# Shashank8834/multimodal-fl-security

Hardware: AMD Instinct MI355X
Metric: FL rounds/sec + aggregate-ms, K=128 clients 10M-param multimodal, 1/2/4/8 GPU (higher is better)
Workload: dtype f32 (bf16x6-split MFMA conv/GEMM = fp32 operands; Krum Gram bf16x4 hi/lo split, fp32 accumulate); 1 GPU; C3: Multi-Krum K=128, 20% sign-flip, ResNet-18 img + 1-layer GRU text late fusion, 5 local SGD steps/round; Krum distances reference-exact; preset=C3, model=resnet18-img+gru1-text late-fusion, clients=128, params=11800394, local_steps=5, batch=32, defense=krum(f=25, multi_k=64), attack=sign_flip, attackers=25, client_chunk=128, exchange=alltoall, krum_distances=reference-exact (fp32 torch.norm accumulation, D bit-identical to krum.py:89-97), training_phase=one captured HIP graph per round; local updates = one flr_train_clients_ex call

## Files before the change

### include/flr.h

```cpp
#ifndef FLR_H
#define FLR_H

#include <stddef.h>
#include <stdint.h>

#ifdef __cplusplus
extern "C" {
#endif

#define FLR_OK 0
#define FLR_ERR_ARG (-1)
#define FLR_ERR_HIP (-2)
#define FLR_ERR_UNSUPPORTED (-3)
#define FLR_ERR_WORKSPACE (-4)
#define FLR_ERR_KRUM_N (-5)

const char* flr_version(void);
const char* flr_build_info(void);
int flr_set_knob(const char* name, const char* value);
const char* flr_status_string(int status);
const char* flr_last_error(void);

size_t flr_pairwise_l2_workspace(int64_t K, int64_t P);
int flr_pairwise_l2(const float* X, int64_t K, int64_t P, int64_t ldx,
// ... 302 lines not shown
                 double* out, void* workspace, size_t workspace_bytes, void* stream);
int flr_weighted_rows(const float* X, int64_t K, int64_t P, int64_t ldx,
                      const int32_t* rows, int64_t m, const float* weights,
                      const float* scales, float divisor, float* out,
                      void* stream);

int flr_gru_fwd_step(const float* gi, const float* gh, float* hseq, float* gates,
                     int64_t K, int64_t B, int64_t T, int64_t H, int64_t t,
                     void* stream);
int flr_gru_bwd_step(const float* dh, const float* gates, const float* hseq,
                     float* dgh, float* dgi, float* dh_direct, int64_t K,
                     int64_t B, int64_t T, int64_t H, int64_t t, void* stream);
int flr_gru_fwd_fused(const float* gi, const float* whhP, const float* bhh, float* hseq, float* gates, int64_t K,
                      int64_t B, int64_t T, int64_t H, int64_t t, void* stream);
int flr_gru_bwd_fused(const float* whhTP, const float* gates, const float* hseq, float* dgh, float* dgi,
                      float* dh_direct, float* dh0, int64_t K, int64_t B, int64_t T, int64_t H, int64_t t,
                      void* stream);
int flr_gru_fwd_fused_ex(const float* gi, const float* whh, int shared_w, const float* bhh,
                         float* hseq, float* gates, int64_t K, int64_t B, int64_t T, int64_t H,
                         int64_t t, void* stream);
int flr_gru_bwd_fused_ex(const float* whhT, int shared_w, const float* gates, const float* hseq,
                         float* dgh, float* dgi, float* dh_direct, float* dh0, int64_t K,
                         int64_t B, int64_t T, int64_t H, int64_t t, void* stream);
int flr_gru_pack(const float* w, int64_t K, int64_t NG, int64_t H, int64_t C, int trans, float* wp, void* stream);

int flr_batchnorm_fwd(const float* x, const float* gamma, const float* beta,
                      const float* residual, float* y, float* mean, float* invstd,
                      int64_t B, int64_t KC, int64_t HW, float eps, int relu,
                      void* stream);
int flr_batchnorm_bwd(const float* dy, const float* x, const float* y,
                      const float* gamma, const float* mean, const float* invstd,
                      float* dx, float* dgamma, float* dbeta, float* dresidual,
                      int64_t B, int64_t KC, int64_t HW, int relu, void* stream);
int flr_batchnorm_relu_maxpool_fwd(const float* x, const float* gamma, const float* beta,
                                   float* y_pool, uint8_t* argmax, float* mean, float* invstd,
                                   int64_t KC, int64_t NI, int64_t H, int64_t W, float eps,
                                   void* stream);
int flr_maxpool_relu_batchnorm_bwd(const float* dy_pool, const uint8_t* argmax, const float* x,
                                   const float* gamma, const float* beta, const float* mean,
                                   const float* invstd, float* dx, float* dgamma, float* dbeta,
                                   int64_t KC, int64_t NI, int64_t H, int64_t W, void* stream);

size_t flr_bgemm_workspace(int64_t batch, int64_t M, int64_t N, int64_t R);
#define FLR_ACT_NONE 0
#define FLR_ACT_RELU 1
#define FLR_ACT_GELU 2
// ... 113 lines not shown
```

### multimodal-fl-security_amd/csrc/train_clients.hip

```cpp
#include "flr_common.h"
#include "side_stream.h"

#include <algorithm>
#include <cstring>
#include <string>
#include <vector>

namespace flr {
int clip_sumsq_blocks(const float* const* g_blocks, const int64_t* numel, const int64_t* client_stride,
                      int64_t nblocks, int64_t K, double* out, int64_t out_ld, int nslots, hipStream_t st);
namespace tc {

constexpr int THREADS = 256;

__global__ void permute_images_kernel(const float* __restrict__ src, float* __restrict__ dst, int64_t K, int64_t B,
                                      int64_t C, int64_t HW) {
  const int64_t n = K * B * C * HW;
  for (int64_t i = (int64_t)blockIdx.x * THREADS + threadIdx.x; i < n; i += (int64_t)gridDim.x * THREADS) {
    const int64_t p = i % HW, r = i / HW;
    const int64_t b = r % B, r2 = r / B;
    const int64_t c = r2 % C, k = r2 / C;
    dst[i] = src[((k * B + b) * C + c) * HW + p];
  }
}
// ... 451 lines not shown
  int step(const float* images, const int64_t* tokens, const int64_t* labels, const float* mask, bool first,
           bool last, float* loss_row, float lr, float mom, hipStream_t st) {
    int rc;
#define FLR_TRY(x) \
  if ((rc = (x)) != FLR_OK) return rc
    const auto& s = s_;
    const int64_t C0 = s.in_channels, HW0 = s.image_size * s.image_size, N = B_ * T_;
    first_ = first;
    hipLaunchKernelGGL(permute_images_kernel, dim3(grid_for(K_ * B_ * C0 * HW0)), dim3(THREADS), 0, st, images,
                       ximg_, K_, B_, C0, HW0);
    FLR_TRY(launch_status("train_clients: images"));
    const Param &emb = ps_[p_emb_], &wih = ps_[p_wih_], &whh = ps_[p_whh_], &bih = ps_[p_bih_],
                &bhh = ps_[p_bhh_], &w1 = ps_[p_w1_], &b1 = ps_[p_b1_], &w2 = ps_[p_w2_], &b2 = ps_[p_b2_];
    const bool conc = text_ != nullptr;
    const hipStream_t ts = conc ? text_->s : st;
    if (conc) FLR_TRY(fork(st, ts, 0));
    FLR_TRY(wait_group(gtext_, ts));
    FLR_TRY(flr_embedding_fwd(emb.w, s.vocab * E_, s.vocab, tokens, N, nullptr, 0, 0, nullptr, 0, nullptr, 0, 0,
                              nullptr, 0, K_, N, E_, emb_, ts));
    const int64_t H3 = 3 * H_;
    FLR_TRY(gemm(emb_, N * E_, E_, 1, wih.w, H3 * E_, E_, 1, gi_, N * H3, H3, 1, bih.w, H3, nullptr, N, H3, E_, ts));
    const bool fused = B_ <= 32;
    const bool wsh = first_ && gshared_ != nullptr;
    if (fused) {
      FLR_TRY(flr_fill(hseq_, K_ * (T_ + 1) * B_ * H_, 0.f, ts));
      FLR_TRY(flr_gru_pack(wsh ? gshared_ + whh.off : whh.w, wsh ? 1 : K_, 3, H_, H_, 0, whhP_, ts));
      for (int64_t t = 0; t < T_; ++t)
        FLR_TRY(flr_gru_fwd_fused_ex(gi_, whhP_, wsh ? 1 : 0, bhh.w, hseq_, gates_, K_, B_, T_, H_, t, ts));
    } else {
      FLR_TRY(flr_fill(hseq_, K_ * (T_ + 1) * B_ * H_, 0.f, ts));
      for (int64_t t = 0; t < T_; ++t) {
        FLR_TRY(gemm(hseq_ + t * B_ * H_, (T_ + 1) * B_ * H_, H_, 1, whh.w, H3 * H_, H_, 1, gh_, B_ * H3, H3, 1,
                     bhh.w, H3, nullptr, B_, H3, H_, ts));
        FLR_TRY(flr_gru_fwd_step(gi_, gh_, hseq_, gates_, K_, B_, T_, H_, t, ts));
      }
    }
    if (conc) FLR_TRY(fork(ts, st, 1));
    int seg = 0;
    FLR_TRY(wait_group(seg++, st));
    FLR_TRY(conv_fwd(stem_, ximg_, y0_, st));
    if (stem_fused_) {
      FLR_TRY(flr_batchnorm_relu_maxpool_fwd(y0_, ps_[stem_bn_.pg].w, ps_[stem_bn_.pb].w, p0_, arg0_, stem_bn_.mean,
                                             stem_bn_.invstd, K_ * s.widths[0], B_, Hs_, Hs_, 1e-5f, st));
    } else {
      FLR_TRY(bn_fwd(stem_bn_, y0_, nullptr, a0_, true, st));
      FLR_TRY(flr_maxpool2d_fwd(a0_, p0_, arg0_, K_ * s.widths[0] * B_, Hs_, Hs_, 3, 3, 2, 1, st));
    }
// ... 35 lines not shown
    FLR_TRY(flr_bgemm_ex(hT, hk, H_, 1, w1.w + Dimg_, F_ * DI, DI, 1, h1_, B_ * F_, F_, 1, nullptr, 0, h1_,
                         FLR_ACT_RELU, mask, nullptr, nullptr, K_, B_, F_, H_, gws_, gws_n_, st));
    FLR_TRY(gemm(h1_, B_ * F_, F_, 1, w2.w, C_ * F_, F_, 1, logits_, B_ * C_, C_, 1, b2.w, C_, nullptr, B_, C_, F_,
                 st));
    FLR_TRY(flr_cross_entropy(logits_, labels, K_, B_, C_, loss_, dlogits_, rows_, st));
    FLR_TRY(flr_copy_rows(loss_, K_, K_, loss_row, K_, 1, st));
    WgradStream* wgs_save = wgs_;
    wev_ = 0;
    FLR_TRY(flr_bgemm_ex(dlogits_, B_ * C_, C_, 1, w2.w, C_ * F_, 1, F_, dpre_, B_ * F_, F_, 1, nullptr, 0, nullptr,
                         FLR_ACT_DRELU, mask, h1_, nullptr, K_, B_, F_, C_, gws_, gws_n_, st));
    FLR_TRY(gemm(dlogits_, B_ * C_, 1, C_, h1_, B_ * F_, 1, F_, w2.g, C_ * F_, F_, 1, nullptr, 0, nullptr, C_, F_, B_,
                 st));
    FLR_TRY(rowsum(dlogits_, B_ * C_, C_, B_, C_, b2.g, st));
    FLR_TRY(gemm(dpre_, B_ * F_, F_, 1, w1.w, F_ * DI, 1, DI, d_x4_, Dimg_ * B_, 1, B_, nullptr, 0, nullptr, B_, Dimg_,
                 F_, st));
    FLR_TRY(gemm(dpre_, B_ * F_, 1, F_, x4, Dimg_ * B_, B_, 1, w1.g, F_ * DI, DI, 1, nullptr, 0, nullptr, F_, Dimg_, B_,
                 st));
    FLR_TRY(gemm(dpre_, B_ * F_, F_, 1, w1.w + Dimg_, F_ * DI, 1, DI, dh_, B_ * H_, H_, 1, nullptr, 0, nullptr, B_, H_,
                 F_, st));
    FLR_TRY(gemm(dpre_, B_ * F_, 1, F_, hT, hk, 1, H_, w1.g + Dimg_, F_ * DI, DI, 1, nullptr, 0, nullptr, F_, H_, B_,
                 st));
    FLR_TRY(rowsum(dpre_, B_ * F_, F_, B_, F_, b1.g, st));
    if (conc) FLR_TRY(fork(st, ts, 2));
    if (fused) {
      FLR_TRY(flr_gru_pack(wsh ? gshared_ + whh.off : whh.w, wsh ? 1 : K_, 1, H_, H3, 1, whhT_, ts));
      FLR_TRY(flr_gru_bwd_step(dh_, gates_, hseq_, dgh_, dgi_, dh_direct_, K_, B_, T_, H_, T_ - 1, ts));
      for (int64_t t = T_ - 1; t > 0; --t)
        FLR_TRY(flr_gru_bwd_fused_ex(whhT_, wsh ? 1 : 0, gates_, hseq_, dgh_, dgi_, dh_direct_, nullptr, K_, B_, T_,
                                     H_, t, ts));
    } else {
      const float* dh = dh_;
      for (int64_t t = T_ - 1; t >= 0; --t) {
        FLR_TRY(flr_gru_bwd_step(dh, gates_, hseq_, dgh_, dgi_, dh_direct_, K_, B_, T_, H_, t, ts));
        if (t > 0) {
          float* out = dh == dh2_ ? dh_ : dh2_;
          FLR_TRY(gemm(dgh_ + t * B_ * H3, T_ * B_ * H3, H3, 1, whh.w, H3 * H_, 1, H_, out, B_ * H_, H_, 1, nullptr,
                       0, dh_direct_, B_, H_, H3, ts));
          dh = out;
        }
      }
    }
    FLR_TRY(gemm(dgh_, T_ * B_ * H3, 1, H3, hseq_, hk, 1, H_, whh.g, H3 * H_, H_, 1, nullptr, 0, nullptr, H3, H_,
                 T_ * B_, ts));
    FLR_TRY(rowsum(dgh_, T_ * B_ * H3, H3, T_ * B_, H3, bhh.g, ts));
    FLR_TRY(gemm(dgi_, N * H3, H3, 1, wih.w, H3 * E_, 1, E_, demb_, N * E_, E_, 1, nullptr, 0, nullptr, N, E_, H3, ts));
    FLR_TRY(gemm(dgi_, N * H3, 1, H3, emb_, N * E_, 1, E_, wih.g, H3 * E_, E_, 1, nullptr, 0, nullptr, H3, E_, N, ts));
    FLR_TRY(rowsum(dgi_, N * H3, H3, N, H3, bih.g, ts));
// ... 475 lines not shown
```

### multimodal-fl-security_amd/csrc/train_gru.hip

```cpp
#include "flr_common.h"

#include <stdlib.h>
#include <string.h>

namespace flr {
namespace gru {

constexpr int THREADS = 256;

__device__ __forceinline__ float sigm(float x) { return 1.0f / (1.0f + expf(-x)); }

struct Dims {
  int K, B, T, H, t;
  int wshared;
};

__device__ __forceinline__ void decompose(const Dims& d, int64_t idx, int& k, int& b, int& j) {
  j = (int)(idx % d.H);
  const int64_t kb = idx / d.H;
  b = (int)(kb % d.B);
  k = (int)(kb / d.B);
}

__global__ __launch_bounds__(THREADS) void fwd_step_kernel(const float* __restrict__ gi, const float* __restrict__ gh,
                                                           float* __restrict__ hseq, float* __restrict__ gates,
                                                           const Dims d) {
  const int64_t idx = (int64_t)blockIdx.x * THREADS + threadIdx.x;
  if (idx >= (int64_t)d.K * d.B * d.H) return;
  int k, b, j;
  decompose(d, idx, k, b, j);
  const int H = d.H;
  const int64_t kb = (int64_t)k * d.B + b;
  const float* gir = gi + (kb * d.T + d.t) * 3 * H;
  const float* ghr = gh + kb * 3 * H;
  const int64_t hrow = (((int64_t)k * (d.T + 1) + d.t) * d.B + b) * H;
  const float hp = hseq[hrow + j];
  const float r = sigm(gir[j] + ghr[j]);
  const float z = sigm(gir[H + j] + ghr[H + j]);
  const float hn = ghr[2 * H + j];
  const float n = tanhf(gir[2 * H + j] + r * hn);
  hseq[hrow + (int64_t)d.B * H + j] = (hp - n) * z + n;
  float* g = gates + (((int64_t)k * d.T + d.t) * d.B + b) * 4 * H;
  g[j] = r;
  g[H + j] = z;
  g[2 * H + j] = n;
  g[3 * H + j] = hn;
}

__global__ __launch_bounds__(THREADS) void bwd_step_kernel(const float* __restrict__ dh,
                                                           const float* __restrict__ gates,
                                                           const float* __restrict__ hseq, float* __restrict__ dgh,
                                                           float* __restrict__ dgi, float* __restrict__ dh_direct,
                                                           const Dims d) {
  const int64_t idx = (int64_t)blockIdx.x * THREADS + threadIdx.x;
  if (idx >= (int64_t)d.K * d.B * d.H) return;
  int k, b, j;
  decompose(d, idx, k, b, j);
  const int H = d.H;
  const int64_t kb = (int64_t)k * d.B + b;
  const int64_t srow = ((int64_t)k * d.T + d.t) * d.B + b;
  const float* g = gates + srow * 4 * H;
  const float r = g[j], z = g[H + j], n = g[2 * H + j], hn = g[3 * H + j];
  const float hp = hseq[(((int64_t)k * (d.T + 1) + d.t) * d.B + b) * H + j];
  const float dy = dh[idx];
  const float dz = dy * (hp - n);
  const float dn = dy * (1.0f - z);
  const float dnp = dn * (1.0f - n * n);
  const float dr = dnp * hn;
  const float drp = dr * (r * (1.0f - r));
  const float dzp = dz * (z * (1.0f - z));
  float* o = dgh + srow * 3 * H;
  o[j] = drp;
  o[H + j] = dzp;
  o[2 * H + j] = dnp * r;
  float* q = dgi + (kb * d.T + d.t) * 3 * H;
  q[j] = drp;
  q[H + j] = dzp;
  q[2 * H + j] = dnp;
  dh_direct[idx] = dy * z;
}

typedef __bf16 bf16x8 __attribute__((ext_vector_type(8)));
typedef float f32x16 __attribute__((ext_vector_type(16)));

__device__ __forceinline__ void split3(const float (&v)[8], bf16x8& hi, bf16x8& mid, bf16x8& lo) {
#pragma unroll
  for (int j = 0; j < 8; ++j) {
    const __bf16 a = (__bf16)v[j];
    const float r1 = v[j] - (float)a;
    const __bf16 b = (__bf16)r1;
    hi[j] = a;
    mid[j] = b;
    lo[j] = (__bf16)(r1 - (float)b);
  }
}

using rsrc_t = __amdgpu_buffer_rsrc_t;
typedef float f32x4 __attribute__((ext_vector_type(4)));
constexpr unsigned SENT = 0x80000000u;

__device__ __forceinline__ rsrc_t make_rsrc(const float* p, int64_t nfloats) {
  const uint64_t a = reinterpret_cast<uint64_t>(p);
  const uint32_t lo = __builtin_amdgcn_readfirstlane((uint32_t)a);
  const uint32_t hi = __builtin_amdgcn_readfirstlane((uint32_t)(a >> 32));
  const int bytes = __builtin_amdgcn_readfirstlane((int)(nfloats * 4));
  void* base = reinterpret_cast<void*>(((uint64_t)hi << 32) | lo);
  return __builtin_amdgcn_make_buffer_rsrc(base, (short)0, bytes, 0x00020000);
}

template <bool V8>
__device__ __forceinline__ void bload8(rsrc_t r, bool ok, int row_off, int k0, int R, float (&v)[8]) {
  if constexpr (V8) {
    const unsigned off = (ok && k0 < R) ? (unsigned)(row_off + k0) * 4u : SENT;
    const f32x4 x = __builtin_bit_cast(f32x4, __builtin_amdgcn_raw_buffer_load_b128(r, off, 0, 0));
    const f32x4 y = __builtin_bit_cast(f32x4, __builtin_amdgcn_raw_buffer_load_b128(r, off + 16u, 0, 0));
    v[0] = x[0]; v[1] = x[1]; v[2] = x[2]; v[3] = x[3];
// ... 114 lines not shown
  } else {
#pragma unroll
    for (int g = 0; g < 3; ++g)
#pragma unroll
      for (int e = 0; e < 16; ++e) red[wave][g][e][lane] = acc[g][e];
    __syncthreads();
  }
#pragma unroll
  for (int i = 0; i < EPT; ++i) {
    const int p = threadIdx.x + 64 * NW * i, e = p >> 6, ln = p & 63;
    const int b = (e & 3) + 8 * (e >> 2) + 4 * (ln >> 5), j = j0 + (ln & 31);
    if (b >= B || j >= H) continue;
    float v[3];
#pragma unroll
    for (int g = 0; g < 3; ++g) {
      float x = red[0][g][e][ln];
      if constexpr (!SEQ)
#pragma unroll
        for (int w = 1; w < NW; ++w) x += red[w][g][e][ln];
      v[g] = x;
    }
    const int64_t hrw = (((int64_t)k * (d.T + 1) + d.t) * B + b) * H;
    const float ghr = pbh[i][0] + v[0], ghz = pbh[i][1] + v[1], hn = pbh[i][2] + v[2];
    const float r = sigm(pgi[i][0] + ghr);
    const float z = sigm(pgi[i][1] + ghz);
    const float n = tanhf(pgi[i][2] + r * hn);
    hseq[hrw + (int64_t)B * H + j] = (php[i] - n) * z + n;
    float* gg = gates + (((int64_t)k * d.T + d.t) * B + b) * 4 * H;
    gg[j] = r;
    gg[H + j] = z;
    gg[2 * H + j] = n;
    gg[3 * H + j] = hn;
  }
}

template <bool V8, int NW, int G, bool SEQ = false>
__global__ __launch_bounds__(64 * NW) __attribute__((amdgpu_waves_per_eu(SEQ ? 6 : 1))) void bwd_fused_kernel(const float* __restrict__ whhTP,
                                                            const float* __restrict__ gates,
                                                            const float* __restrict__ hseq, float* __restrict__ dgh,
                                                            float* __restrict__ dgi, float* __restrict__ dh_direct,
                                                            float* __restrict__ dh0, const Dims d, int nub) {
  constexpr int EPT = 16 / NW;
  __shared__ float red[SEQ ? 1 : NW][16][64];
  int k, ub;
  block_coords(nub, k, ub);
  const int i0 = ub * 32;
  const int wave = threadIdx.x >> 6, lane = threadIdx.x & 63, l32 = lane & 31, h = lane >> 5;
  const int B = d.B, H = d.H, R = 3 * H;
  const int t = d.t + 1;
  const rsrc_t ra = make_rsrc(dgh + ((int64_t)k * d.T + t) * B * R, (int64_t)B * R);
  const int S = (R + 15) / 16, per = (S + NW - 1) / NW;
  const rsrc_t rb = make_rsrc(whhTP + (d.wshared ? 0 : (int64_t)k * nub * S * 512), (int64_t)nub * S * 512);
  const rsrc_t rdd = make_rsrc(dh_direct + (int64_t)k * B * H, (int64_t)B * H);
  const bool elem = d.t >= 0;
// ... 44 lines not shown
#pragma unroll
        for (int e = 0; e < 16; ++e) red[0][e][lane] = w == 0 ? acc[e] : red[0][e][lane] + acc[e];
      __syncthreads();
    }
  } else {
#pragma unroll
    for (int e = 0; e < 16; ++e) red[wave][e][lane] = acc[e];
    __syncthreads();
  }
#pragma unroll
  for (int i = 0; i < EPT; ++i) {
    const int p = threadIdx.x + 64 * NW * i, e = p >> 6, ln = p & 63;
    const int b = (e & 3) + 8 * (e >> 2) + 4 * (ln >> 5), j = i0 + (ln & 31);
    if (b >= B || j >= H) continue;
    float x = red[0][e][ln];
    if constexpr (!SEQ)
#pragma unroll
      for (int w = 1; w < NW; ++w) x += red[w][e][ln];
    const int64_t kb = (int64_t)k * B + b;
    const int64_t idx = kb * H + j;
    const float dy = pdd[i] + x;
    if (dh0) dh0[idx] = dy;
    if (!elem) continue;
    const float r = pg[i][0], z = pg[i][1], n = pg[i][2], hn = pg[i][3];
    const float dz = dy * (php[i] - n);
    const float dn = dy * (1.0f - z);
    const float dnp = dn * (1.0f - n * n);
    const float dr = dnp * hn;
    const float drp = dr * (r * (1.0f - r));
    const float dzp = dz * (z * (1.0f - z));
    const int64_t srow = ((int64_t)k * d.T + d.t) * B + b;
    float* o = dgh + srow * 3 * H;
    o[j] = drp;
    o[H + j] = dzp;
    o[2 * H + j] = dnp * r;
    float* q = dgi + (kb * d.T + d.t) * 3 * H;
    q[j] = drp;
    q[H + j] = dzp;
    q[2 * H + j] = dnp;
    dh_direct[idx] = dy * z;
  }
}

template <int TRANS>
__global__ __launch_bounds__(256) void pack_kernel(const float* __restrict__ w, int NG, int H, int C,
                                                   float* __restrict__ wp) {
  __shared__ float tile[32][129];
  const int k = blockIdx.z, blk = blockIdx.y, c0 = blockIdx.x * 128;
  const int nub = (H + 31) / 32, S = (C + 15) / 16;
  const int g = blk / nub, r0 = (blk % nub) * 32;
  const float* src = w + (int64_t)k * NG * H * C;
  for (int e = threadIdx.x; e < 32 * 128; e += 256) {
    int r, c;
    if (TRANS) { c = e >> 5; r = e & 31; } else { r = e >> 7; c = e & 127; }
    const bool ok = r0 + r < H && c0 + c < C;
    const int64_t off = TRANS ? (int64_t)(c0 + c) * H + r0 + r : ((int64_t)g * H + r0 + r) * C + c0 + c;
    tile[r][c] = ok ? src[off] : 0.f;
  }
  __syncthreads();
  float* dst = wp + ((int64_t)k * NG * nub + blk) * S * 512;
  for (int o = threadIdx.x; o < 8 * 512; o += 256) {
    const int sl = o >> 9, q = (o >> 8) & 1, lane = (o >> 2) & 63, e = o & 3;
    const int s = c0 / 16 + sl;
    if (s < S) dst[(int64_t)s * 512 + q * 256 + lane * 4 + e] = tile[lane & 31][sl * 16 + 8 * (lane >> 5) + 4 * q + e];
  }
}

inline bool dims_ok(int64_t K, int64_t B, int64_t T, int64_t H, int64_t t) {
  return K > 0 && B > 0 && T > 0 && H > 0 && t >= 0 && t < T && K * B * H < (int64_t)1 << 31;
}

}
}

using namespace flr;

extern "C" int flr_gru_fwd_step(const float* gi, const float* gh, float* hseq, float* gates, int64_t K, int64_t B,
                                int64_t T, int64_t H, int64_t t, void* stream) {
  if (!gi || !gh || !hseq || !gates || !gru::dims_ok(K, B, T, H, t)) return FLR_ERR_ARG;
  const gru::Dims d{(int)K, (int)B, (int)T, (int)H, (int)t};
  const int64_t n = K * B * H;
  hipLaunchKernelGGL(gru::fwd_step_kernel, dim3((unsigned)((n + gru::THREADS - 1) / gru::THREADS)),
                     dim3(gru::THREADS), 0, as_stream(stream), gi, gh, hseq, gates, d);
  return launch_status("gru fwd step");
}

extern "C" int flr_gru_bwd_step(const float* dh, const float* gates, const float* hseq, float* dgh, float* dgi,
                                float* dh_direct, int64_t K, int64_t B, int64_t T, int64_t H, int64_t t,
// ... 64 lines not shown
                                 float* dh_direct, float* dh0, int64_t K, int64_t B, int64_t T, int64_t H, int64_t t,
                                 void* stream) {
  return flr_gru_bwd_fused_ex(whhT, 0, gates, hseq, dgh, dgi, dh_direct, dh0, K, B, T, H, t, stream);
}

extern "C" int flr_gru_bwd_fused_ex(const float* whhT, int shared_w, const float* gates, const float* hseq,
                                    float* dgh, float* dgi, float* dh_direct, float* dh0, int64_t K, int64_t B,
                                    int64_t T, int64_t H, int64_t t, void* stream) {
  if (!whhT || !gates || !hseq || !dgh || !dgi || !dh_direct || !gru::dims_ok(K, B, T, H, t) || t < 1 || B > 32 ||
      K > 65535)
    return FLR_ERR_ARG;
  const gru::Dims d{(int)K, (int)B, (int)T, (int)H, (int)(t - 1), shared_w ? 1 : 0};
  const int nub = (int)((H + 31) / 32);
  const int cfg = gru::cfg_index("FLR_GRU_BW", 1);
  if (H % 8 == 0)
    gru::launch_bwd<true>(cfg, dim3((unsigned)(K * nub)), as_stream(stream), whhT, gates, hseq, dgh, dgi, dh_direct,
                          dh0, d, nub);
  else
    gru::launch_bwd<false>(cfg, dim3((unsigned)(K * nub)), as_stream(stream), whhT, gates, hseq, dgh, dgi, dh_direct,
                           dh0, d, nub);
  return launch_status("gru bwd fused");
}

extern "C" int flr_gru_pack(const float* w, int64_t K, int64_t NG, int64_t H, int64_t C, int trans, float* wp,
                            void* stream) {
  if (!w || !wp || K < 1 || K > 65535 || NG < 1 || H < 1 || C < 1 || (trans && NG != 1) ||
      K * NG * H * C >= (int64_t)1 << 31)
    return FLR_ERR_ARG;
  const dim3 grid((unsigned)((C + 127) / 128), (unsigned)(NG * ((H + 31) / 32)), (unsigned)K);
  if (trans)
    hipLaunchKernelGGL(gru::pack_kernel<1>, grid, dim3(256), 0, as_stream(stream), w, (int)NG, (int)H, (int)C, wp);
  else
    hipLaunchKernelGGL(gru::pack_kernel<0>, grid, dim3(256), 0, as_stream(stream), w, (int)NG, (int)H, (int)C, wp);
  return launch_status("gru pack");
}
```

### multimodal-fl-security_amd/flr/_capi.py

```python
from __future__ import annotations

import ctypes
import os
import threading

import torch

_PKG_ROOT = os.path.dirname(os.path.dirname(os.path.abspath(__file__)))
LIB_PATH = os.environ.get("FLR_LIB", os.path.join(_PKG_ROOT, "lib", "libflr.so"))
HEADER_PATH = os.path.join(os.path.dirname(_PKG_ROOT), "include", "flr.h")

FLR_OK = 0
FLR_ERR_ARG = -1
FLR_ERR_HIP = -2
FLR_ERR_UNSUPPORTED = -3
FLR_ERR_WORKSPACE = -4
FLR_ERR_KRUM_N = -5

_c_void_p = ctypes.c_void_p
_i64 = ctypes.c_int64
_size_t = ctypes.c_size_t
_int = ctypes.c_int

SIGNATURES = {
# ... 174 lines not shown
    "flr_layernorm_fwd": (_int, [_c_void_p, _i64, _c_void_p, _i64, _c_void_p, _c_void_p, _c_void_p, _i64, _c_void_p,
                                 _i64, _c_void_p, _c_void_p, _i64, _i64, _i64, ctypes.c_float, _c_void_p]),
    "flr_layernorm_bwd_workspace": (_size_t, [_i64, _i64, _i64]),
    "flr_layernorm_bwd": (_int, [_c_void_p, _i64, _c_void_p, _i64, _c_void_p, _c_void_p, _c_void_p, _c_void_p, _i64,
                                 _c_void_p, _i64, _c_void_p, _c_void_p, _i64, _i64, _i64, _c_void_p, _size_t,
                                 _c_void_p]),
    "flr_vit_tokens": (_int, [_c_void_p, _c_void_p, _c_void_p, _i64, _i64, _i64, _i64, _c_void_p, _c_void_p]),
    "flr_attention_fwd": (_int, [_c_void_p, _i64, _i64, _i64, _i64, _c_void_p, _c_void_p, _c_void_p]),
    "flr_attention_bwd": (_int, [_c_void_p, _c_void_p, _c_void_p, _c_void_p, _i64, _i64, _i64, _i64, _c_void_p,
                                 _c_void_p]),
    "flr_sum_rows": (_int, [_c_void_p, _i64, _i64, _i64, _i64, _i64, _c_void_p, _i64, _c_void_p]),
    "flr_sum_rows_workspace": (_size_t, [_i64, _i64, _i64]),
    "flr_sum_rows_ex": (_int, [_c_void_p, _i64, _i64, _i64, _i64, _i64, _c_void_p, _i64, _c_void_p, _size_t,
                               _c_void_p]),
    "flr_maxpool2d_fwd": (_int, [_c_void_p] * 3 + [_i64] * 7 + [_c_void_p]),
    "flr_maxpool2d_bwd": (_int, [_c_void_p] * 3 + [_i64] * 7 + [_c_void_p]),
    "flr_gru_fwd_step": (_int, [_c_void_p] * 4 + [_i64] * 5 + [_c_void_p]),
    "flr_gru_bwd_step": (_int, [_c_void_p] * 6 + [_i64] * 5 + [_c_void_p]),
    "flr_gru_fwd_fused": (_int, [_c_void_p] * 5 + [_i64] * 5 + [_c_void_p]),
    "flr_gru_bwd_fused": (_int, [_c_void_p] * 7 + [_i64] * 5 + [_c_void_p]),
    "flr_gru_pack": (_int, [_c_void_p, _i64, _i64, _i64, _i64, _int, _c_void_p, _c_void_p]),
    "flr_gru_fwd_fused_ex": (_int, [_c_void_p, _c_void_p, _int] + [_c_void_p] * 3 + [_i64] * 5 + [_c_void_p]),
    "flr_gru_bwd_fused_ex": (_int, [_c_void_p, _int] + [_c_void_p] * 6 + [_i64] * 5 + [_c_void_p]),
    "flr_batchnorm_infer": (_int, [_c_void_p] * 7 + [_i64, _i64, ctypes.c_float, _int, _c_void_p]),
    "flr_classify_rows": (_int, [_c_void_p, _c_void_p, _i64, _i64, _i64, _i64, _c_void_p, _c_void_p, _c_void_p,
                                 _c_void_p]),
}

_lock = threading.Lock()
_lib = None


class FlrError(RuntimeError):

    def __init__(self, fn: str, status: int, detail: str = ""):
        self.status = status
        msg = f"{fn} failed: {status_string(status)} ({status})"
        if detail:
            msg += f": {detail}"
        super().__init__(msg)


def lib() -> ctypes.CDLL:
    global _lib
    if _lib is not None:
        return _lib
    with _lock:
# ... 52 lines not shown
```

Measured before the change: 16.95 rounds/s.

## Fuse GRU time loop into one persistent kernel per client for fwd and bwd

Adds sequence-level GRU forward and backward kernels that run all timesteps inside one block per client. The recurrent state is kept in double-buffered LDS as a bf16 hi/mid/lo split, and the recurrent weights are streamed with software-pipelined buffer loads. This replaces T per-step kernel launches and their global round-trips of the hidden state, and zeroes only h0 rather than filling the whole hseq buffer. It is enabled when K*(H/32) exceeds 768 or when a knob forces it. The trade-off is that each client is limited to one workgroup, which can cap parallelism on small K.

After: 17.32 rounds/s, median of 6. 2.1% higher.

```diff
diff --git a/include/flr.h b/include/flr.h
--- a/include/flr.h
+++ b/include/flr.h
@@ -348,6 +348,14 @@
 int flr_gru_bwd_fused_ex(const float* whhT, int shared_w, const float* gates, const float* hseq,
                          float* dgh, float* dgi, float* dh_direct, float* dh0, int64_t K,
                          int64_t B, int64_t T, int64_t H, int64_t t, void* stream);
+int flr_gru_fwd_seq(const float* gi, const float* whhP, int shared_w, const float* bhh, float* hseq, float* gates,
+                    int64_t K, int64_t B, int64_t T, int64_t H, void* stream);
+int flr_gru_bwd_seq(const float* whhTP, int shared_w, const float* gates, const float* hseq, const float* dh,
+                    float* dgh, float* dgi, float* dh_direct, float* dh0, int64_t K, int64_t B, int64_t T,
+                    int64_t H, void* stream);
+int flr_gru_seq_supported(int64_t K, int64_t B, int64_t T, int64_t H);
+int flr_gru_seq_preferred(int64_t K, int64_t B, int64_t T, int64_t H);
+int flr_gru_zero_h0(float* hseq, int64_t K, int64_t B, int64_t T, int64_t H, void* stream);
 int flr_gru_pack(const float* w, int64_t K, int64_t NG, int64_t H, int64_t C, int trans, float* wp, void* stream);
 
 int flr_batchnorm_fwd(const float* x, const float* gamma, const float* beta,
diff --git a/multimodal-fl-security_amd/csrc/train_clients.hip b/multimodal-fl-security_amd/csrc/train_clients.hip
--- a/multimodal-fl-security_amd/csrc/train_clients.hip
+++ b/multimodal-fl-security_amd/csrc/train_clients.hip
@@ -497,7 +497,12 @@
     FLR_TRY(gemm(emb_, N * E_, E_, 1, wih.w, H3 * E_, E_, 1, gi_, N * H3, H3, 1, bih.w, H3, nullptr, N, H3, E_, ts));
     const bool fused = B_ <= 32;
     const bool wsh = first_ && gshared_ != nullptr;
-    if (fused) {
+    const bool seq = fused && flr_gru_seq_preferred(K_, B_, T_, H_) != 0;
+    if (seq) {
+      FLR_TRY(flr_gru_zero_h0(hseq_, K_, B_, T_, H_, ts));
+      FLR_TRY(flr_gru_pack(wsh ? gshared_ + whh.off : whh.w, wsh ? 1 : K_, 3, H_, H_, 0, whhP_, ts));
+      FLR_TRY(flr_gru_fwd_seq(gi_, whhP_, wsh ? 1 : 0, bhh.w, hseq_, gates_, K_, B_, T_, H_, ts));
+    } else if (fused) {
       FLR_TRY(flr_fill(hseq_, K_ * (T_ + 1) * B_ * H_, 0.f, ts));
       FLR_TRY(flr_gru_pack(wsh ? gshared_ + whh.off : whh.w, wsh ? 1 : K_, 3, H_, H_, 0, whhP_, ts));
       for (int64_t t = 0; t < T_; ++t)
@@ -579,7 +584,11 @@
                  st));
     FLR_TRY(rowsum(dpre_, B_ * F_, F_, B_, F_, b1.g, st));
     if (conc) FLR_TRY(fork(st, ts, 2));
-    if (fused) {
+    if (seq) {
+      FLR_TRY(flr_gru_pack(wsh ? gshared_ + whh.off : whh.w, wsh ? 1 : K_, 1, H_, H3, 1, whhT_, ts));
+      FLR_TRY(flr_gru_bwd_seq(whhT_, wsh ? 1 : 0, gates_, hseq_, dh_, dgh_, dgi_, dh_direct_, nullptr, K_, B_, T_, H_,
+                              ts));
+    } else if (fused) {
       FLR_TRY(flr_gru_pack(wsh ? gshared_ + whh.off : whh.w, wsh ? 1 : K_, 1, H_, H3, 1, whhT_, ts));
       FLR_TRY(flr_gru_bwd_step(dh_, gates_, hseq_, dgh_, dgi_, dh_direct_, K_, B_, T_, H_, T_ - 1, ts));
       for (int64_t t = T_ - 1; t > 0; --t)
diff --git a/multimodal-fl-security_amd/csrc/train_gru.hip b/multimodal-fl-security_amd/csrc/train_gru.hip
--- a/multimodal-fl-security_amd/csrc/train_gru.hip
+++ b/multimodal-fl-security_amd/csrc/train_gru.hip
@@ -9,6 +9,35 @@
 constexpr int THREADS = 256;
 
 __device__ __forceinline__ float sigm(float x) { return 1.0f / (1.0f + expf(-x)); }
+
+struct Gate {
+  float r, z, n, h;
+};
+__device__ __forceinline__ Gate gate_math(float gir, float giz, float gin, float ghr, float ghz, float hn, float hp) {
+  Gate o;
+  o.r = sigm(gir + ghr);
+  o.z = sigm(giz + ghz);
+  o.n = tanhf(gin + o.r * hn);
+  o.h = (hp - o.n) * o.z + o.n;
+  return o;
+}
+
+struct ElemBwd {
+  float drp, dzp, dnp, dnr, dhd;
+};
+__device__ __forceinline__ ElemBwd elem_bwd(float dy, float r, float z, float n, float hn, float hp) {
+  const float dz = dy * (hp - n);
+  const float dn = dy * (1.0f - z);
+  const float dnp = dn * (1.0f - n * n);
+  const float dr = dnp * hn;
+  ElemBwd o;
+  o.drp = dr * (r * (1.0f - r));
+  o.dzp = dz * (z * (1.0f - z));
+  o.dnp = dnp;
+  o.dnr = dnp * r;
+  o.dhd = dy * z;
+  return o;
+}
 
 struct Dims {
   int K, B, T, H, t;
@@ -35,15 +64,13 @@
   const float* ghr = gh + kb * 3 * H;
   const int64_t hrow = (((int64_t)k * (d.T + 1) + d.t) * d.B + b) * H;
   const float hp = hseq[hrow + j];
-  const float r = sigm(gir[j] + ghr[j]);
-  const float z = sigm(gir[H + j] + ghr[H + j]);
   const float hn = ghr[2 * H + j];
-  const float n = tanhf(gir[2 * H + j] + r * hn);
-  hseq[hrow + (int64_t)d.B * H + j] = (hp - n) * z + n;
+  const Gate o = gate_math(gir[j], gir[H + j], gir[2 * H + j], ghr[j], ghr[H + j], hn, hp);
+  hseq[hrow + (int64_t)d.B * H + j] = o.h;
   float* g = gates + (((int64_t)k * d.T + d.t) * d.B + b) * 4 * H;
-  g[j] = r;
-  g[H + j] = z;
-  g[2 * H + j] = n;
+  g[j] = o.r;
+  g[H + j] = o.z;
+  g[2 * H + j] = o.n;
   g[3 * H + j] = hn;
 }
 
@@ -62,36 +89,36 @@
   const float* g = gates + srow * 4 * H;
   const float r = g[j], z = g[H + j], n = g[2 * H + j], hn = g[3 * H + j];
   const float hp = hseq[(((int64_t)k * (d.T + 1) + d.t) * d.B + b) * H + j];
-  const float dy = dh[idx];
-  const float dz = dy * (hp - n);
-  const float dn = dy * (1.0f - z);
-  const float dnp = dn * (1.0f - n * n);
-  const float dr = dnp * hn;
-  const float drp = dr * (r * (1.0f - r));
-  const float dzp = dz * (z * (1.0f - z));
+  const ElemBwd eb = elem_bwd(dh[idx], r, z, n, hn, hp);
   float* o = dgh + srow * 3 * H;
-  o[j] = drp;
-  o[H + j] = dzp;
-  o[2 * H + j] = dnp * r;
+  o[j] = eb.drp;
+  o[H + j] = eb.dzp;
+  o[2 * H + j] = eb.dnr;
   float* q = dgi + (kb * d.T + d.t) * 3 * H;
-  q[j] = drp;
-  q[H + j] = dzp;
-  q[2 * H + j] = dnp;
-  dh_direct[idx] = dy * z;
+  q[j] = eb.drp;
+  q[H + j] = eb.dzp;
+  q[2 * H + j] = eb.dnp;
+  dh_direct[idx] = eb.dhd;
 }
 
 typedef __bf16 bf16x8 __attribute__((ext_vector_type(8)));
 typedef float f32x16 __attribute__((ext_vector_type(16)));
 
+__device__ __forceinline__ void split1(float v, __bf16& hi, __bf16& mid, __bf16& lo) {
+  hi = (__bf16)v;
+  const float r1 = v - (float)hi;
+  mid = (__bf16)r1;
+  lo = (__bf16)(r1 - (float)mid);
+}
+
 __device__ __forceinline__ void split3(const float (&v)[8], bf16x8& hi, bf16x8& mid, bf16x8& lo) {
 #pragma unroll
   for (int j = 0; j < 8; ++j) {
-    const __bf16 a = (__bf16)v[j];
-    const float r1 = v[j] - (float)a;
-    const __bf16 b = (__bf16)r1;
+    __bf16 a, b, c;
+    split1(v[j], a, b, c);
     hi[j] = a;
     mid[j] = b;
-    lo[j] = (__bf16)(r1 - (float)b);
+    lo[j] = c;
   }
 }
 
@@ -252,14 +279,12 @@
     }
     const int64_t hrw = (((int64_t)k * (d.T + 1) + d.t) * B + b) * H;
     const float ghr = pbh[i][0] + v[0], ghz = pbh[i][1] + v[1], hn = pbh[i][2] + v[2];
-    const float r = sigm(pgi[i][0] + ghr);
-    const float z = sigm(pgi[i][1] + ghz);
-    const float n = tanhf(pgi[i][2] + r * hn);
-    hseq[hrw + (int64_t)B * H + j] = (php[i] - n) * z + n;
+    const Gate o = gate_math(pgi[i][0], pgi[i][1], pgi[i][2], ghr, ghz, hn, php[i]);
+    hseq[hrw + (int64_t)B * H + j] = o.h;
     float* gg = gates + (((int64_t)k * d.T + d.t) * B + b) * 4 * H;
-    gg[j] = r;
-    gg[H + j] = z;
-    gg[2 * H + j] = n;
+    gg[j] = o.r;
+    gg[H + j] = o.z;
+    gg[2 * H + j] = o.n;
     gg[3 * H + j] = hn;
   }
 }
@@ -350,23 +375,17 @@
     const float dy = pdd[i] + x;
     if (dh0) dh0[idx] = dy;
     if (!elem) continue;
-    const float r = pg[i][0], z = pg[i][1], n = pg[i][2], hn = pg[i][3];
-    const float dz = dy * (php[i] - n);
-    const float dn = dy * (1.0f - z);
-    const float dnp = dn * (1.0f - n * n);
-    const float dr = dnp * hn;
-    const float drp = dr * (r * (1.0f - r));
-    const float dzp = dz * (z * (1.0f - z));
+    const ElemBwd eb = elem_bwd(dy, pg[i][0], pg[i][1], pg[i][2], pg[i][3], php[i]);
     const int64_t srow = ((int64_t)k * d.T + d.t) * B + b;
     float* o = dgh + srow * 3 * H;
-    o[j] = drp;
-    o[H + j] = dzp;
-    o[2 * H + j] = dnp * r;
+    o[j] = eb.drp;
+    o[H + j] = eb.dzp;
+    o[2 * H + j] = eb.dnr;
     float* q = dgi + (kb * d.T + d.t) * 3 * H;
-    q[j] = drp;
-    q[H + j] = dzp;
-    q[2 * H + j] = dnp;
-    dh_direct[idx] = dy * z;
+    q[j] = eb.drp;
+    q[H + j] = eb.dzp;
+    q[2 * H + j] = eb.dnp;
+    dh_direct[idx] = eb.dhd;
   }
 }
 
@@ -392,6 +411,280 @@
     const int s = c0 / 16 + sl;
     if (s < S) dst[(int64_t)s * 512 + q * 256 + lane * 4 + e] = tile[lane & 31][sl * 16 + 8 * (lane >> 5) + 4 * q + e];
   }
+}
+
+constexpr int SEQ_NW = 8;
+constexpr int SEQ_HMAX = 256;
+
+__device__ __forceinline__ int tile_row(int e, int h) { return (e & 3) + 8 * (e >> 2) + 4 * h; }
+
+template <int NG_, int NUB_, int S_>
+struct SeqGeo {
+  static constexpr int NG = NG_, NUB = NUB_, S = S_;
+  static constexpr int PER = (S + SEQ_NW - 1) / SEQ_NW;
+  static constexpr int RS = 16 * S + 8;
+  static constexpr int IMG = 96 * RS;
+};
+template <class G>
+using WBuf = float[G::PER][G::NG][8];
+
+template <class G, int W>
+__device__ __forceinline__ void wload(rsrc_t rw, unsigned voff, WBuf<G>& v) {
+#pragma unroll
+  for (int q = 0; q < G::PER; ++q) {
+    const int s = W * G::PER + q;
+    if (s < G::S) {
+#pragma unroll
+      for (int g = 0; g < G::NG; ++g) {
+        const int soff = ((g * G::NUB * G::S + s) * 512) * 4;
+        const f32x4 x = __builtin_bit_cast(f32x4, __builtin_amdgcn_raw_buffer_load_b128(rw, voff, soff, 0));
+        const f32x4 y = __builtin_bit_cast(f32x4, __builtin_amdgcn_raw_buffer_load_b128(rw, voff, soff + 1024, 0));
+        v[q][g][0] = x[0]; v[q][g][1] = x[1]; v[q][g][2] = x[2]; v[q][g][3] = x[3];
+        v[q][g][4] = y[0]; v[q][g][5] = y[1]; v[q][g][6] = y[2]; v[q][g][7] = y[3];
+      }
+    }
+  }
+}
+
+template <class G, int W>
+__device__ __forceinline__ void wmma(const __bf16* a, const WBuf<G>& v, f32x16 (&x)[G::NG]) {
+  f32x16 p[G::NG];
+#pragma unroll
+  for (int g = 0; g < G::NG; ++g)
+#pragma unroll
+    for (int e = 0; e < 16; ++e) p[g][e] = 0.f;
+#pragma unroll
+  for (int q = 0; q < G::PER; ++q) {
+    const int s = W * G::PER + q;
+    if (s < G::S) {
+      const bf16x8 ah = *reinterpret_cast<const bf16x8*>(a + 16 * s);
+      const bf16x8 am = *reinterpret_cast<const bf16x8*>(a + 16 * s + 32 * G::RS);
+      const bf16x8 al = *reinterpret_cast<const bf16x8*>(a + 16 * s + 64 * G::RS);
+#pragma unroll
+      for (int g = 0; g < G::NG; ++g) {
+        bf16x8 bh, bm, bl;
+        split3(v[q][g], bh, bm, bl);
+        p[g] = mfma6(ah, am, al, bh, bm, bl, p[g]);
+      }
+      __builtin_amdgcn_sched_barrier(0);
+    }
+  }
+#pragma unroll
+  for (int g = 0; g < G::NG; ++g)
+#pragma unroll
+    for (int e = 0; e < 16; ++e) x[g][e] = W == 0 ? p[g][e] : x[g][e] + p[g][e];
+#pragma unroll
+  for (int g = 0; g < G::NG; ++g) asm volatile("" : "+v"(x[g]));
+}
+
+template <class G>
+__device__ __forceinline__ void img_put(__bf16* p, int off, float v) {
+  __bf16 a, b, c;
+  split1(v, a, b, c);
+  p[off] = a;
+  p[off + 32 * G::RS] = b;
+  p[off + 64 * G::RS] = c;
+}
+
+template <class G, int W = 0, class Last>
+__device__ __forceinline__ void wgemm(const __bf16* a, rsrc_t rw, unsigned voff, WBuf<G>& bA, WBuf<G>& bB,
+                                      f32x16 (&x)[G::NG], Last last) {
+  wload<G, W + 1>(rw, voff, bB);
+  __builtin_amdgcn_sched_barrier(0);
+  wmma<G, W>(a, bA, x);
+  __builtin_amdgcn_sched_barrier(0);
+  if constexpr (W + 2 < SEQ_NW)
+    wload<G, W + 2>(rw, voff, bA);
+  else
+    last();
+  __builtin_amdgcn_sched_barrier(0);
+  wmma<G, W + 1>(a, bB, x);
+  __builtin_amdgcn_sched_barrier(0);
+  if constexpr (W + 2 < SEQ_NW) wgemm<G, W + 2>(a, rw, voff, bA, bB, x, last);
+}
+
+__device__ __forceinline__ float ldg(rsrc_t r, unsigned voff, int soff) {
+  return __builtin_bit_cast(float, __builtin_amdgcn_raw_buffer_load_b32(r, voff, soff, 0));
+}
+__device__ __forceinline__ void stg(rsrc_t r, float v, unsigned voff, int soff) {
+  __builtin_amdgcn_raw_buffer_store_b32(__builtin_bit_cast(unsigned, v), r, voff, soff, 0);
+}
+__device__ __forceinline__ unsigned per_step(unsigned v) {
+  asm volatile("" : "+v"(v));
+  return v;
+}
+
+template <int H>
+__global__ __launch_bounds__(2 * H) void fwd_seq_kernel(const float* __restrict__ gi, const float* __restrict__ whhP,
+                                                        const float* __restrict__ bhh, float* __restrict__ hseq,
+                                                        float* __restrict__ gates, const Dims d) {
+  using G = SeqGeo<3, H / 32, H / 16>;
+  __shared__ __attribute__((aligned(16))) __bf16 img[2 * G::IMG];
+  const int k = blockIdx.x, ub = __builtin_amdgcn_readfirstlane(threadIdx.x >> 6), lane = threadIdx.x & 63;
+  const int l32 = lane & 31, h = lane >> 5, j = ub * 32 + l32;
+  const int B = d.B, T = d.T;
+  for (int i = threadIdx.x * 8; i < 2 * G::IMG; i += 2 * H * 8)
+    *reinterpret_cast<f32x4*>(img + i) = f32x4{0.f, 0.f, 0.f, 0.f};
+  __syncthreads();
+  constexpr int64_t WN = (int64_t)3 * G::NUB * G::S * 512;
+  const rsrc_t rw = make_rsrc(whhP + (d.wshared ? 0 : k * WN) + ub * G::S * 512, WN - ub * G::S * 512);
+  const rsrc_t rg = make_rsrc(gi + (int64_t)k * B * T * 3 * H, (int64_t)B * T * 3 * H);
+  const rsrc_t rbias = make_rsrc(bhh + (int64_t)k * 3 * H, (int64_t)3 * H);
+  const rsrc_t rh = make_rsrc(hseq + (int64_t)k * (T + 1) * B * H, (int64_t)(T + 1) * B * H);
+  const rsrc_t rgt = make_rsrc(gates + (int64_t)k * T * B * 4 * H, (int64_t)T * B * 4 * H);
+  const unsigned voff = lane * 16;
+  const unsigned vgi = (4 * h * T * 3 * H + j) * 4, vh = (4 * h * H + j) * 4, vgt = (4 * h * 4 * H + j) * 4;
+  WBuf<G> bA, bB;
+  wload<G, 0>(rw, voff, bA);
+  float hp[16], pbh[3];
+#pragma unroll
+  for (int g = 0; g < 3; ++g) pbh[g] = bload1(rbias, true, g * H + j);
+#pragma unroll
+  for (int e = 0; e < 16; ++e) {
+    const int b = tile_row(e, h);
+    hp[e] = ldg(rh, b < B ? vh : SENT, tile_row(e, 0) * H * 4);
+    if (b < B) img_put<G>(img + 4 * h * G::RS + j, tile_row(e, 0) * G::RS, hp[e]);
+  }
+  __syncthreads();
+  for (int t = 0; t < T; ++t) {
+    const __bf16* cur = img + (t & 1) * G::IMG + l32 * G::RS + 8 * h;
+    __bf16* nxt = img + ((t + 1) & 1) * G::IMG + 4 * h * G::RS + j;
+    f32x16 x[3];
+    float pgi[16][3];
+    wgemm<G>(cur, rw, voff, bA, bB, x, [&]() {
+      const unsigned v = per_step(vgi);
+#pragma unroll
+      for (int e = 0; e < 16; ++e) {
+        const unsigned off = tile_row(e, h) < B ? v : SENT;
+#pragma unroll
+        for (int g = 0; g < 3; ++g) pgi[e][g] = ldg(rg, off + g * H * 4, ((tile_row(e, 0) * T + t) * 3 * H) * 4);
+      }
+    });
+    wload<G, 0>(rw, voff, bA);
+    __builtin_amdgcn_sched_barrier(0);
+#pragma unroll
+    for (int e = 0; e < 16; ++e) {
+      const int b = tile_row(e, h);
+      if (b < B) {
+        const float ghr = pbh[0] + x[0][e], ghz = pbh[1] + x[1][e], hn = pbh[2] + x[2][e];
+        const Gate o = gate_math(pgi[e][0], pgi[e][1], pgi[e][2], ghr, ghz, hn, hp[e]);
+        stg(rh, o.h, vh, (((t + 1) * B + tile_row(e, 0)) * H) * 4);
+        const int sg = ((t * B + tile_row(e, 0)) * 4 * H) * 4;
+        stg(rgt, o.r, vgt, sg);
+        stg(rgt, o.z, vgt + H * 4, sg);
+        stg(rgt, o.n, vgt + 2 * H * 4, sg);
+        stg(rgt, hn, vgt + 3 * H * 4, sg);
+        hp[e] = o.h;
+        img_put<G>(nxt, tile_row(e, 0) * G::RS, o.h);
+      }
+      __builtin_amdgcn_sched_barrier(0);
+    }
+    __syncthreads();
+  }
+}
+
+template <int H>
+__global__ __launch_bounds__(2 * H) void bwd_seq_kernel(const float* __restrict__ whhTP,
+                                                        const float* __restrict__ gates,
+                                                        const float* __restrict__ hseq, const float* __restrict__ dh,
+                                                        float* __restrict__ dgh, float* __restrict__ dgi,
+                                                        float* __restrict__ dh_direct, float* __restrict__ dh0,
+                                                        const Dims d) {
+  using G = SeqGeo<1, H / 32, 3 * H / 16>;
+  constexpr int R = 3 * H;
+  __shared__ __attribute__((aligned(16))) __bf16 img[G::IMG];
+  const int k = blockIdx.x, ub = __builtin_amdgcn_readfirstlane(threadIdx.x >> 6), lane = threadIdx.x & 63;
+  const int l32 = lane & 31, h = lane >> 5, j = ub * 32 + l32;
+  const int B = d.B, T = d.T;
+  for (int i = threadIdx.x * 8; i < G::IMG; i += 2 * H * 8)
+    *reinterpret_cast<f32x4*>(img + i) = f32x4{0.f, 0.f, 0.f, 0.f};
+  __syncthreads();
+  constexpr int64_t WN = (int64_t)G::NUB * G::S * 512;
+  const rsrc_t rw = make_rsrc(whhTP + (d.wshared ? 0 : k * WN) + ub * G::S * 512, WN - ub * G::S * 512);
+  const rsrc_t rgt = make_rsrc(gates + (int64_t)k * T * B * 4 * H, (int64_t)T * B * 4 * H);
+  const rsrc_t rhp = make_rsrc(hseq + (int64_t)k * (T + 1) * B * H, (int64_t)(T + 1) * B * H);
+  const rsrc_t rdgh = make_rsrc(dgh + (int64_t)k * T * B * R, (int64_t)T * B * R);
+  const rsrc_t rdgi = make_rsrc(dgi + (int64_t)k * B * T * R, (int64_t)B * T * R);
+  const rsrc_t rdd = make_rsrc(dh_direct + (int64_t)k * B * H, (int64_t)B * H);
+  const rsrc_t rdh0 = make_rsrc(dh0 ? dh0 + (int64_t)k * B * H : nullptr, dh0 ? (int64_t)B * H : 0);
+  const unsigned vh = (4 * h * H + j) * 4, vgt = (4 * h * 4 * H + j) * 4, vgh = (4 * h * R + j) * 4;
+  const unsigned vgi = (4 * h * T * R + j) * 4;
+  float pg[16][4], php[16];
+  auto load_epi = [&](int t) {
+    const unsigned v4 = per_step(vgt), v1 = per_step(vh);
+#pragma unroll
+    for (int e = 0; e < 16; ++e) {
+      const bool ok = tile_row(e, h) < B;
+      const int rowt = t * B + tile_row(e, 0);
+#pragma unroll
+      for (int q = 0; q < 4; ++q) pg[e][q] = ldg(rgt, (ok ? v4 : SENT) + q * H * 4, rowt * 4 * H * 4);
+      php[e] = ldg(rhp, ok ? v1 : SENT, rowt * H * 4);
+    }
+  };
+  float dd[16];
+  auto elem = [&](int t, int e, float dy) {
+    const ElemBwd eb = elem_bwd(dy, pg[e][0], pg[e][1], pg[e][2], pg[e][3], php[e]);
+    const int so = ((t * B + tile_row(e, 0)) * R) * 4, si = ((tile_row(e, 0) * T + t) * R) * 4;
+    stg(rdgh, eb.drp, vgh, so);
+    stg(rdgh, eb.dzp, vgh + H * 4, so);
+    stg(rdgh, eb.dnr, vgh + 2 * H * 4, so);
+    stg(rdgi, eb.drp, vgi, si);
+    stg(rdgi, eb.dzp, vgi + H * 4, si);
+    stg(rdgi, eb.dnp, vgi + 2 * H * 4, si);
+    dd[e] = eb.dhd;
+    if (t == 0) {
+      stg(rdd, eb.dhd, vh, tile_row(e, 0) * H * 4);
+    } else {
+      __bf16* p = img + 4 * h * G::RS + j;
+      img_put<G>(p, tile_row(e, 0) * G::RS, eb.drp);
+      img_put<G>(p, tile_row(e, 0) * G::RS + H, eb.dzp);
+      img_put<G>(p, tile_row(e, 0) * G::RS + 2 * H, eb.dnr);
+    }
+  };
+  load_epi(T - 1);
+  {
+    const rsrc_t rdh = make_rsrc(dh + (int64_t)k * B * H, (int64_t)B * H);
+#pragma unroll
+    for (int e = 0; e < 16; ++e) {
+      const bool ok = tile_row(e, h) < B;
+      const float dy = ldg(rdh, ok ? vh : SENT, tile_row(e, 0) * H * 4);
+      if (ok) elem(T - 1, e, dy);
+    }
+  }
+  if (T < 2) return;
+  const unsigned voff = lane * 16;
+  const __bf16* a = img + l32 * G::RS + 8 * h;
+  WBuf<G> bA, bB;
+  wload<G, 0>(rw, voff, bA);
+  __syncthreads();
+  for (int t = T - 1; t >= 1; --t) {
+    f32x16 x[1];
+    wgemm<G>(a, rw, voff, bA, bB, x, [&]() { load_epi(t - 1); });
+    wload<G, 0>(rw, voff, bA);
+    __builtin_amdgcn_sched_barrier(0);
+    __syncthreads();
+#pragma unroll
+    for (int e = 0; e < 16; ++e) {
+      if (tile_row(e, h) < B) {
+        const float dy = dd[e] + x[0][e];
+        if (dh0 && t == 1) stg(rdh0, dy, vh, tile_row(e, 0) * H * 4);
+        elem(t - 1, e, dy);
+      }
+      __builtin_amdgcn_sched_barrier(0);
+    }
+    __syncthreads();
+  }
+}
+
+__global__ __launch_bounds__(THREADS) void zero_h0_kernel(float* __restrict__ hseq, int64_t n, int64_t stride) {
+  const int64_t i = (int64_t)blockIdx.x * THREADS + threadIdx.x;
+  if (i < n) hseq[(int64_t)blockIdx.y * stride + i] = 0.f;
+}
+
+inline bool seq_shape_ok(int64_t K, int64_t B, int64_t T, int64_t H) {
+  const char* e = flr::knob("FLR_GRU_SEQ");
+  if (e && e[0] == '0') return false;
+  return B <= 32 && H % 32 == 0 && H <= SEQ_HMAX && 32 * (T + 1) * 4 * H < (int64_t)1 << 29;
 }
 
 inline bool dims_ok(int64_t K, int64_t B, int64_t T, int64_t H, int64_t t) {
@@ -502,6 +795,56 @@
   return launch_status("gru bwd fused");
 }
 
+extern "C" int flr_gru_seq_supported(int64_t K, int64_t B, int64_t T, int64_t H) {
+  return K > 0 && K <= 65535 && B > 0 && T > 0 && H > 0 && gru::seq_shape_ok(K, B, T, H) ? 1 : 0;
+}
+
+extern "C" int flr_gru_seq_preferred(int64_t K, int64_t B, int64_t T, int64_t H) {
+  if (!flr_gru_seq_supported(K, B, T, H)) return 0;
+  const char* e = flr::knob("FLR_GRU_SEQ");
+  return (e && e[0] == '1') || K * (H / 32) > 3 * 256 ? 1 : 0;
+}
+
+extern "C" int flr_gru_zero_h0(float* hseq, int64_t K, int64_t B, int64_t T, int64_t H, void* stream) {
+  if (!hseq || K < 1 || K > 65535 || B < 1 || T < 1 || H < 1 || B * H >= (int64_t)1 << 31) return FLR_ERR_ARG;
+  const int64_t n = B * H;
+  hipLaunchKernelGGL(gru::zero_h0_kernel, dim3((unsigned)((n + gru::THREADS - 1) / gru::THREADS), (unsigned)K),
+                     dim3(gru::THREADS), 0, as_stream(stream), hseq, n, (T + 1) * n);
+  return launch_status("gru zero h0");
+}
+
+extern "C" int flr_gru_fwd_seq(const float* gi, const float* whhP, int shared_w, const float* bhh, float* hseq,
+                               float* gates, int64_t K, int64_t B, int64_t T, int64_t H, void* stream) {
+  if (!gi || !whhP || !bhh || !hseq || !gates || !gru::dims_ok(K, B, T, H, 0) || K > 65535) return FLR_ERR_ARG;
+  if (!gru::seq_shape_ok(K, B, T, H)) return FLR_ERR_UNSUPPORTED;
+  const gru::Dims d{(int)K, (int)B, (int)T, (int)H, 0, shared_w ? 1 : 0};
+  switch (H / 32) {
+#define FLR_SEQ_CASE(N) \
+  case N: hipLaunchKernelGGL(gru::fwd_seq_kernel<32 * N>, dim3((unsigned)K), dim3(64 * N), 0, as_stream(stream), gi, whhP, bhh, hseq, gates, d); break;
+    FLR_SEQ_CASE(1) FLR_SEQ_CASE(2) FLR_SEQ_CASE(3) FLR_SEQ_CASE(4) FLR_SEQ_CASE(5) FLR_SEQ_CASE(6) FLR_SEQ_CASE(7)
+    FLR_SEQ_CASE(8)
+#undef FLR_SEQ_CASE
+  }
+  return launch_status("gru fwd seq");
+}
+
+extern "C" int flr_gru_bwd_seq(const float* whhTP, int shared_w, const float* gates, const float* hseq,
+                               const float* dh, float* dgh, float* dgi, float* dh_direct, float* dh0, int64_t K,
+                               int64_t B, int64_t T, int64_t H, void* stream) {
+  if (!whhTP || !gates || !hseq || !dh || !dgh || !dgi || !dh_direct || !gru::dims_ok(K, B, T, H, 0) || K > 65535)
+    return FLR_ERR_ARG;
+  if (!gru::seq_shape_ok(K, B, T, H)) return FLR_ERR_UNSUPPORTED;
+  const gru::Dims d{(int)K, (int)B, (int)T, (int)H, 0, shared_w ? 1 : 0};
+  switch (H / 32) {
+#define FLR_SEQ_CASE(N) \
+  case N: hipLaunchKernelGGL(gru::bwd_seq_kernel<32 * N>, dim3((unsigned)K), dim3(64 * N), 0, as_stream(stream), whhTP, gates, hseq, dh, dgh, dgi, dh_direct, dh0, d); break;
+    FLR_SEQ_CASE(1) FLR_SEQ_CASE(2) FLR_SEQ_CASE(3) FLR_SEQ_CASE(4) FLR_SEQ_CASE(5) FLR_SEQ_CASE(6) FLR_SEQ_CASE(7)
+    FLR_SEQ_CASE(8)
+#undef FLR_SEQ_CASE
+  }
+  return launch_status("gru bwd seq");
+}
+
 extern "C" int flr_gru_pack(const float* w, int64_t K, int64_t NG, int64_t H, int64_t C, int trans, float* wp,
                             void* stream) {
   if (!w || !wp || K < 1 || K > 65535 || NG < 1 || H < 1 || C < 1 || (trans && NG != 1) ||
diff --git a/multimodal-fl-security_amd/flr/_capi.py b/multimodal-fl-security_amd/flr/_capi.py
--- a/multimodal-fl-security_amd/flr/_capi.py
+++ b/multimodal-fl-security_amd/flr/_capi.py
@@ -220,7 +220,12 @@
     "flr_gru_pack": (_int, [_c_void_p, _i64, _i64, _i64, _i64, _int, _c_void_p, _c_void_p]),
     "flr_gru_fwd_fused_ex": (_int, [_c_void_p, _c_void_p, _int] + [_c_void_p] * 3 + [_i64] * 5 + [_c_void_p]),
     "flr_gru_bwd_fused_ex": (_int, [_c_void_p, _int] + [_c_void_p] * 6 + [_i64] * 5 + [_c_void_p]),
-    "flr_batchnorm_infer": (_int, [_c_void_p] * 7 + [_i64, _i64, ctypes.c_float, _int, _c_void_p]),
+    "flr_gru_fwd_seq": (_int, [_c_void_p, _c_void_p, _int] + [_c_void_p] * 3 + [_i64] * 4 + [_c_void_p]),
+    "flr_gru_bwd_seq": (_int, [_c_void_p, _int] + [_c_void_p] * 7 + [_i64] * 4 + [_c_void_p]),
+    "flr_gru_seq_supported": (_int, [_i64] * 4),
+    "flr_gru_seq_preferred": (_int, [_i64] * 4),
+    "flr_gru_zero_h0": (_int, [_c_void_p] + [_i64] * 4 + [_c_void_p]),
+    "flr_batchnorm_infer":(_int, [_c_void_p] * 7 + [_i64, _i64, ctypes.c_float, _int, _c_void_p]),
     "flr_classify_rows": (_int, [_c_void_p, _c_void_p, _i64, _i64, _i64, _i64, _c_void_p, _c_void_p, _c_void_p,
                                  _c_void_p]),
 }
```
